# david8862/tf-keras-speech-commands

Hardware: AMD Instinct MI355X
Metric: 1 s@16 kHz clips/sec train-step, simple_cnn bs4096, 1/2/4/8 MI355X; eval top-1 (higher is better)
Workload: dtype f32; 1 GPU; configs[1]: simple_cnn train step = featurize(f32 1 s @16 kHz) + fwd + bwd + Adam, 36 logits (background + 35 words), batch 4096 per GPU; global_batch=4096, parallelism=dp1, gradient_exchange=none (one rank), rccl_ranks=0, library_build=546ca62dfe01

## Files before the change

### tf-keras-speech-commands_amd/csrc/kws_cnn_plan.h

```cpp
#pragma once
#include "kws_model_types.h"
#include "kws_layers.h"
#include "kws_layer1.h"
#include "kws_infer_fused.h"
#include "kws_conv_group.h"
#include "kws_dense_head.h"

namespace kws {

struct CnnPlan {
    bool training, bf16, det;
    bool prepared;
    bool fused_tail;
    bool group;
    bool dense_fused;
    bool l1m;
    bool l1_default_map;
    bool prep_in_stats;
    bool l1_conv2;
    bool compact_g2;
    bool routed_g2;
    bool fuse_pool2;
    bool acc_fwd;
    bool acc_bn2, acc_bn3, acc_bn4;
    bool a3_on_load;
    bool pool4_fused;
    bool wgrad2_bf16;
    bool wgrad2_early;
    bool l1_fin_in_kernel;
    bool head_bwd_fuses;
    bool fuse_head_fwd;
};

inline CnnPlan plan_cnn(const kws_model *m, int B, int mprec, bool training, bool capturing, bool wants_head_outputs, bool prepared)
{
    const CnnDims &d = m->d;
    CnnPlan p{};
    p.training = training;
    p.bf16 = mprec == 1;
    p.det = m->deterministic != 0;
    p.prepared = !training && prepared;
    const bool split_train = p.bf16 && training;
    const bool default_tail = m->kind == KWS_SIMPLE_CNN && d.H2 == kFuH2 && d.W2 == kFuW2 && d.H3 == kFuH3 && d.W3 == kFuW3;
    p.fused_tail = !training && wants_head_outputs && p.bf16 && default_tail && d.H4 == kFuH4 && d.W4 == kFuW4 && m->C <= kFuHeadCols;
    p.group = split_train && default_tail && (long)blocks_for(B, kFuClips) <= kStatStride;
    p.head_bwd_fuses = head_bwd_fuses(m);
    p.fuse_head_fwd = p.head_bwd_fuses && !p.det;
    p.dense_fused = split_train && m->kind == KWS_SIMPLE_CNN && p.fuse_head_fwd && m->head_K == kDhK && d.flat % (16 * kDhWaves) == 0 && d.flat <= 1024;
    p.l1m = d.H0 % 2 == 0 && d.W0 % 2 == 0 && (d.H0 + 2) * (d.W0 + 2) <= 64 * kL1Stage && (d.H0 / 2) * (d.W0 / 2) <= 4 * kL1MaxTiles;
    p.l1_default_map = d.H0 == 30 && d.W0 == 20;
    p.prep_in_stats = split_train && p.l1m;
    const int P1 = d.H1 * d.W1;
    p.compact_g2 = p.bf16 && P1 * 8 <= 1280 && (size_t)(d.H1 / 2) * (d.W1 / 2) * 32 <= sizeof(float) * (size_t)d.H3 * d.W3 * 64;
    p.routed_g2 = p.compact_g2;
    p.fuse_pool2 = p.group && p.routed_g2 && d.H1 == kGrH1 && d.W1 == kGrW1;
    const bool acc_ok = !p.det && !capturing;
    p.acc_fwd = p.fuse_pool2 && acc_ok;
    p.l1_conv2 = p.prep_in_stats && p.acc_fwd && p.l1_default_map;
    p.a3_on_load = split_train;
    p.pool4_fused = p.acc_fwd && p.dense_fused;
    p.wgrad2_bf16 = p.bf16 && P1 <= 160;
    p.wgrad2_early = p.compact_g2 && p.wgrad2_bf16 && P1 * 8 <= 1280 && P1 * 4 <= 768;
    p.acc_bn2 = p.group && acc_ok && p.routed_g2 && p.wgrad2_early;
    p.acc_bn3 = p.group && acc_ok;
    p.acc_bn4 = p.dense_fused && acc_ok && d.flat == d.H4 * d.W4 * kDhK;
    p.l1_fin_in_kernel = acc_ok && p.l1_default_map;
    return p;
}

}
```

### tf-keras-speech-commands_amd/csrc/kws_model.hip

```cpp
#include <cstdlib>
#include <cstring>
#include <string>
#include <vector>

#include "kws_common.h"
#include "kws_model_types.h"
#include "kws_conv.h"
#include "kws_layers.h"
#include "kws_layer1.h"
#include "kws_layer1_moments.h"
#include "kws_layer1_fast.h"
#include "kws_l1_conv2.h"
#include "kws_lite.h"
#include "kws_lite_f16.h"
#include "kws_infer_fused.h"
#include "kws_conv_group.h"
#include "kws_dense_head.h"
#include "kws_cnn_plan.h"

using namespace kws;

namespace {

inline int same_out(int n, int s) { return (n + s - 1) / s; }
inline int same_pad_before(int n, int k, int s)
{
    const int out = same_out(n, s), total = std::max((out - 1) * s + k - n, 0);
    return total / 2;
}

struct OverlapHook {
    hipEvent_t ev = nullptr;
    void (*cb)(void *) = nullptr;
    void *user = nullptr;
    int at = 0;
    bool fired = false;
    bool wants(int point) const { return !fired && point == at; }
    int fire(int point, hipStream_t s, bool already_bound = false)
    {
        if (fired || point != at) return KWS_OK;
        fired = true;
        if (ev && !already_bound) KWS_HIP_CHECK(hipEventRecord(ev, s));
        if (cb) cb(user);
        return KWS_OK;
    }
};

#define KWS_TRY_NB(...)               \
    do {                              \
        const int rc__ = (__VA_ARGS__); \
        if (rc__ < 0) return rc__;    \
    } while (0)
#define KWS_TRY(...)                  \
    do {                              \
        if (int rc__ = (__VA_ARGS__)) return rc__; \
    } while (0)

constexpr int kCh[5] = {1, 16, 32, 64, 128};
constexpr int kMaxStatBlocks = kStatStride;

struct CnnWs {
    float *z[4], *a[4], *d1, *loss_i, *correct_i, *dlogits, *dd1, *da4, *gz[4], *da[3];
    float *dwo[4], *ddw[4];
    float *coef[4];
    __bf16 *wsp[3][6];
    __bf16 *dzp[3];
    double *partial;
    double *moments;
    float *zmax2;
    unsigned char *arg2;
    float *zmax4;
    unsigned char *arg4;
    unsigned char *base;
    size_t bytes;
};

CnnWs carve_cnn(const kws_model *m, int B, bool training, unsigned char *base)
{
    CnnWs w{};
    w.base = base;
    size_t off = 0;
    auto take = [&](size_t nfloats) {
        float *p = reinterpret_cast<float *>(base + off);
        off = al256(off + nfloats * sizeof(float));
        return p;
    };
    const CnnDims &d = m->d;
    const size_t zs[4] = {(size_t)d.H0 * d.W0 * 16, (size_t)d.H1 * d.W1 * 32, (size_t)d.H3 * d.W3 * 64, (size_t)d.H3 * d.W3 * 128};
    const size_t as[4] = {(size_t)d.H1 * d.W1 * 16, (size_t)d.H2 * d.W2 * 32, (size_t)d.H3 * d.W3 * 64, (size_t)d.flat};
    const bool lite = m->kind == KWS_SIMPLE_CNN_LITE;
    const size_t dws[4] = {(size_t)d.H0 * d.W0 * 1, (size_t)d.H1 * d.W1 * 16, (size_t)d.H3 * d.W3 * 32, (size_t)d.H3 * d.W3 * 64};
    for (int i = 0; i < 4; ++i) { w.z[i] = take((i == 0 && !lite) ? 0 : zs[i] * B); w.a[i] = take(as[i] * B); }
    for (int i = 0; i < 4; ++i) w.dwo[i] = take(lite ? dws[i] * B : 0);
    w.d1 = take((size_t)B * 128);
    w.loss_i = take(B);
    w.correct_i = take(B);
    for (int i = 0; i < 4; ++i) w.coef[i] = take(6 * 128);
    {
        const size_t wn[3] = {(size_t)9 * 32 * 64, (size_t)9 * 64 * 128, (size_t)d.flat * 128};
        for (int t = 0; t < 3; ++t)
            for (int q = 0; q < 6; ++q) w.wsp[t][q] = reinterpret_cast<__bf16 *>(take(lite ? 0 : (wn[t] + 1) / 2));
    }
    w.partial = reinterpret_cast<double *>(take((size_t)kMaxStatBlocks * 9 * 64 * 2));
    w.moments = reinterpret_cast<double *>(take(2 * kMomCount));
    if (training) {
        w.dlogits = take((size_t)B * m->C);
        w.dd1 = take((size_t)B * 128);
        w.da4 = take((size_t)B * d.flat);
        for (int i = 0; i < 4; ++i) w.gz[i] = take((i == 0 && !lite) ? 0 : zs[i] * B);
        for (int p = 0; p < 3; ++p) w.dzp[p] = reinterpret_cast<__bf16 *>(take(lite ? 0 : (zs[3] * B + 1) / 2));
        for (int i = 0; i < 4; ++i) w.ddw[i] = take(lite ? dws[i] * B : 0);
        for (int i = 0; i < 3; ++i) w.da[i] = take(as[i] * B);
        w.zmax2 = take(lite ? 0 : as[1] * B);
        w.arg2 = reinterpret_cast<unsigned char *>(take(lite ? 0 : (as[1] * B + 3) / 4));
        w.zmax4 = take(lite ? 0 : as[3] * B);
        w.arg4 = reinterpret_cast<unsigned char *>(take(lite ? 0 : (as[3] * B + 3) / 4));
    }
    w.bytes = off;
    return w;
}

BnCoef coef_of(float *base, int C) { return BnCoef{base, base + C, base + 2 * C, base + 3 * C, base + 4 * C, base + 5 * C}; }
static double *acc_set(ModelRes *R, int pass, int layer, unsigned parity) { return R->acc + ((size_t)(pass * 4 + layer) * 2 + (parity & 1u)) * kAccDoubles; }
static int acc_make_clean(ModelRes *R, hipStream_t s)
{
    if (R->acc_dirty) {
        KWS_HIP_CHECK(hipMemsetAsync(R->acc, 0, sizeof(double) * 2 * 4 * 2 * kAccDoubles, s));
        R->acc_dirty = false;
    }
    return KWS_OK;
}

static int infer_coefs(const kws_model *m, const float *params, const float *state, CnnWs &w, hipStream_t s)
{
    BnInferAll a;
    for (int l = 0; l < 4; ++l) {
        a.C[l] = kCh[l + 1];
        a.gamma[l] = params + m->o_g[l]; a.beta[l] = params + m->o_b[l];
        a.mm[l] = state + m->o_mm[l]; a.mv[l] = state + m->o_mv[l];
        a.k[l] = coef_of(w.coef[l], kCh[l + 1]);
    }
    KWS_LAUNCH("bn_infer_coef_all_kernel", bn_infer_coef_all_kernel, dim3(4), dim3(128), 0, s, a);
    return KWS_OK;
}

inline void stat_grid(long M, int C, int &nblk, int &rows)
{
    const int R = 256 / C;
    long want = (M + (long)R * 8 - 1) / ((long)R * 8);
    nblk = (int)std::min<long>(kMaxStatBlocks, std::max<long>(1, want));
    rows = (int)((M + nblk - 1) / nblk);
    nblk = (int)((M + rows - 1) / rows);
}

template <int CR, int CO, int MODE, int EPI>
int launch_gemm(const float *src, const float *w, const float *bias, float *dst, const ConvGeom &g, hipStream_t s)
{
    const long M = (long)g.B * g.Ho * g.Wo;
    static const std::string name = std::string("conv_gemm_fwd<") + std::to_string(CR) + "," +
                                    std::to_string(CO) + ">";
    KWS_LAUNCH(name.c_str(), (conv_gemm_kernel<CR, CO, MODE, EPI>), dim3(blocks_for(M, 64)), dim3(256), 0, s, src, w, bias, dst, g);
    return KWS_OK;
}

static int cu_count() { return device_cus(); }
// ... 598 lines not shown
    } else
        KWS_TRY(run_head_bwd(m, B, params, w.d1, w.dlogits, w.dd1, grads, true, s, nullptr, w.loss_i, w.correct_i,
                             stats, P.det));
    const bool fork0_bound = stop_event_bound(fork0_ev);
    if (P.fuse_head_fwd) {
        if (a->forward_event) KWS_HIP_CHECK(hipEventRecord(static_cast<hipEvent_t>(a->forward_event), s));
        if (hook) KWS_TRY(hook->fire(1, s));
    }
    const ConvGeom g = dense_geom(d, B);
    const bool hook_ev_here = hook && hook->wants(2) && hook->ev;
    if (hook) KWS_TRY(hook->fire(2, s, fork0_bound && hook_ev_here));
    if (hook_ev_here) {
        KWS_HIP_CHECK(hipStreamWaitEvent(s2, fork0_ev, 0));
    } else {
        if (!fork0_bound) KWS_HIP_CHECK(hipEventRecord(R->ev[0], s));
        KWS_HIP_CHECK(hipStreamWaitEvent(s2, R->ev[0], 0));
    }
    if (P.fuse_head_fwd && stats) KWS_LAUNCH("loss_reduce_kernel", loss_reduce_kernel, dim3(1), dim3(256), 0, s2, w.loss_i, w.correct_i, B, stats);
    KWS_TRY(launch_wgrad<128, 128, 1>(w.a[3], w.dd1, grads + m->o_dk, g, s2, P.det));
    if (!P.fuse_head_fwd) {
        int nblk, rows;
        stat_grid(B, 128, nblk, rows);
        KWS_LAUNCH("channel_stats_kernel.dense", channel_stats_kernel, dim3(nblk), dim3(256), 0, s, w.dd1, (long)B, 128, rows, w.partial);
        KWS_LAUNCH("colsum_finalize_kernel", colsum_finalize_kernel, dim3(128), dim3(256), 0, s, w.partial, nblk, 128, grads + m->o_db);
    }
    if (P.dense_fused) ;
    else if (P.bf16) KWS_TRY_NB(launch_bf16<128, 128, MODE_DGRAD, EPI_NONE>("conv_bf16_dgrad", w.dd1, w.wsp[2], nullptr, w.da4, g, s));
    else KWS_TRY(launch_dgrad<128, 128, 1>(w.dd1, params + m->o_dk, w.da4, g, s));
    if (hook) KWS_TRY(hook->fire(3, s));
    return KWS_OK;
}

int CnnCtx::bwd_layer4()
{
    const int C = 128, H = d.H3, W = d.W3;
    const long M = pixels(3);
    const BnCoef k = coef(3);
    const float *gamma = params + m->o_g[3];
    const float rate = drop_rate();
    int nblk, rows;
    stat_grid((long)B * (H / 2) * (W / 2), C, nblk, rows);
    if (P.acc_bn4) ;
    else if (P.bf16)
        KWS_LAUNCH(prof_name("bn_bwd_reduce_pool_kernel", 4), bn_bwd_reduce_routed_full_kernel, dim3(nblk), dim3(256), 0, s, w.zmax4, w.arg4, w.da4, k,
                   w.gz[3], B, H, W, C, rows, w.partial, rate, slo(), shi());
    else KWS_TRY(bwd_reduce_pool(3, H, W, C, w.da4, rate, nblk, rows));
    if (!P.acc_bn4) KWS_TRY(bwd_bn_finalize(3, C, nblk));
    bwd_arm(3);
    const Bf16PlanesOut dzp{{w.dzp[0], w.dzp[1], w.dzp[2]}};
    if (P.acc_bn4)
        KWS_LAUNCH(prof_name("bn_bwd_apply_planes_kernel", 4), bn_bwd_apply_routed_planes_kernel<true>, dim3(std::min<unsigned>(1024u, blocks_for(M * C / 4, 256))),
                   dim3(256), 0, s, w.z[3], w.da4, w.arg4, k, gamma, B, H, W, C, acc_out(3), dzp);
    else if (P.bf16)
        KWS_LAUNCH(prof_name("bn_bwd_apply_planes_kernel", 4), bn_bwd_apply_planes_kernel<true>, dim3(blocks_for(M * C / 4, 256)), dim3(256), 0, s,
                   w.z[3], w.gz[3], k, gamma, M * C / 4, C, dzp);
    else
        KWS_LAUNCH(prof_name("bn_bwd_apply_kernel", 4), bn_bwd_apply_kernel<true>, dim3(blocks_for(M * C, 256)), dim3(256), 0, s, w.z[3], w.gz[3], k,
                   gamma, M * C, C);
    if (hook) KWS_TRY(hook->fire(4, s));
    KWS_TRY(bwd_fork(3));
    const float *in = w.a[2], *kern = params + m->o_k[3];
    float *dk = grads + m->o_k[3];
    const ConvGeom g = geom3x3(B, H, W, 1);
    if (P.bf16 && P.a3_on_load)
        KWS_TRY((launch_wgrad_bf16<64, 128, 1, true, true>(w.z[2], nullptr, dk, g, s2, w.dzp, P.det, coef(2).scale)));
    else if (P.bf16) KWS_TRY(launch_wgrad_bf16<64, 128, 1, true>(in, nullptr, dk, g, s2, w.dzp, P.det));
    else KWS_TRY(launch_wgrad<64, 128, 1>(in, w.gz[3], dk, g, s2, P.det));
    if (a->comm) KWS_TRY(comm_allreduce_early(a->comm, grads + m->o_k[3], m->P - m->o_k[3], s2));
    if (a->bucket_event) KWS_HIP_CHECK(hipEventRecord(static_cast<hipEvent_t>(a->bucket_event), s2));
    if (P.group) {
        fused_bn3_blocks = launch_group_dgrad4(m, B, w, s, P.acc_bn3 ? acc_set(R, 1, 2, bpar[2]) : nullptr);
        if (fused_bn3_blocks < 0) return fused_bn3_blocks;
    } else if (P.bf16 && blocks_for(M, 64) <= (unsigned)kStatStride) {
        const BnCoef k3 = coef(2);
        fused_bn3_blocks = launch_bf16<128, 64, MODE_DGRAD, EPI_BNBWD_GATE6>("conv_bf16_dgrad", nullptr, w.wsp[1], k3.scale, w.gz[2], g, s, w.partial,
                                                                             w.z[2], w.dzp);
        if (fused_bn3_blocks < 0) return fused_bn3_blocks;
    } else if (P.bf16)
        KWS_TRY_NB(launch_bf16<128, 64, MODE_DGRAD, EPI_NONE>("conv_bf16_dgrad", nullptr, w.wsp[1], nullptr, w.da[2], g, s, nullptr, nullptr, w.dzp));
    else KWS_TRY(launch_dgrad<128, 64, 1>(w.gz[3], kern, w.da[2], g, s));
    return KWS_OK;
}

int CnnCtx::bwd_layer3()
{
    const int C = 64, H = d.H3, W = d.W3;
    if (hook) KWS_TRY(hook->fire(5, s));
    const long M = pixels(2);
    const BnCoef k = coef(2);
    const float *gamma = params + m->o_g[2];
    int nblk, rows;
    stat_grid(M, C, nblk, rows);
    if (fused_bn3_blocks > 0) nblk = fused_bn3_blocks;
    else
        KWS_LAUNCH(prof_name("bn_bwd_reduce_kernel", 3), bn_bwd_reduce_kernel<false>, dim3(nblk), dim3(256), 0, s, w.z[2], w.da[2], k, w.gz[2], B, H, W, C,
                   rows, w.partial, 0.f, slo(), shi());
    if (!P.acc_bn3) KWS_TRY(bwd_bn_finalize(2, C, nblk));
    bwd_arm(2);
    if (P.acc_bn3)
        KWS_LAUNCH(prof_name("bn_bwd_apply_kernel", 3), bn_bwd_apply_acc_kernel<false>, dim3(std::min<unsigned>(1024u, blocks_for(M * C / 4, 256))), dim3(256), 0, s,
                   w.z[2], w.gz[2], k, gamma, M * C / 4, C, acc_out(2));
    else
        KWS_LAUNCH(prof_name("bn_bwd_apply_kernel", 3), bn_bwd_apply_kernel<false>, dim3(blocks_for(M * C, 256)), dim3(256), 0, s, w.z[2], w.gz[2], k,
                   gamma, M * C, C);
    KWS_TRY(bwd_fork(2));
    const float *in = w.a[1], *kern = params + m->o_k[2];
    float *dk = grads + m->o_k[2];
    const ConvGeom g = geom3x3(B, d.H2, d.W2, 2);
    if (P.bf16) KWS_TRY(launch_wgrad_bf16<32, 64, 3>(in, w.gz[2], dk, g, s2, nullptr, P.det));
    else KWS_TRY(launch_wgrad<32, 64, 3>(in, w.gz[2], dk, g, s2, P.det));
    if (P.group) {
        if (P.acc_bn2) bwd_arm(1);
        KWS_TRY(launch_group_dgrad3(m, B, w, s, P.acc_bn2 ? acc_set(R, 1, 1, bpar[1]) : nullptr));
    }
    else KWS_TRY(launch_dgrad<64, 32, 2>(w.gz[2], kern, w.da[1], g, s));
    return KWS_OK;
}

int CnnCtx::bwd_layer2()
{
    const int C = 32, H1 = d.H1, W1 = d.W1;
    const long M = pixels(1);
    const BnCoef k = coef(1);
    const long NW = (long)B * (H1 / 2) * (W1 / 2);
    int nblk, rows;
    stat_grid(NW, C, nblk, rows);
    if (P.acc_bn2) ;
    else if (P.compact_g2 && P.routed_g2)
        KWS_LAUNCH(prof_name("bn_bwd_reduce_pool_kernel", 2), bn_bwd_reduce_routed_kernel, dim3(nblk), dim3(256), 0, s, w.zmax2, w.da[1], k, NW, C,
                   rows, w.partial);
    else if (P.compact_g2)
        KWS_LAUNCH(prof_name("bn_bwd_reduce_pool_kernel", 2), bn_bwd_reduce_pool_kernel<true>, dim3(nblk), dim3(256), 0, s, w.z[1], w.da[1], k,
                   w.gz[1], B, H1, W1, C, rows, w.partial, 0.f, slo(), shi(), reinterpret_cast<unsigned char *>(w.da[2]));
    else KWS_TRY(bwd_reduce_pool(1, H1, W1, C, w.da[1], 0.f, nblk, rows));
    if (!P.acc_bn2) {
        if (P.wgrad2_early) bwd_arm(1);
        KWS_TRY(bwd_bn_finalize(1, C, nblk));
    }
    const float *in = w.a[0], *kern = params + m->o_k[1];
    float *dk = grads + m->o_k[1];
    const Conv2Clip cc = conv2_clip(d, B);
    BnBwdArgs bn = {w.z[1], params + m->o_g[1], k.mean, k.inv, k.k2, k.k3};
    if (P.compact_g2) { bn.gw = w.da[1]; bn.arg = P.routed_g2 ? w.arg2 : reinterpret_cast<const unsigned char *>(w.da[2]); }
    BnBwdArgs bn_w = bn;
    if (P.acc_bn2) {
        bn.acc = bn_w.acc = acc_set(R, 1, 1, bpar[1]);
        bn.M = bn_w.M = M;
        bn.acc_clear_set = acc_set(R, 1, 1, bpar[1] + 1);
        bn.dgamma = grads + m->o_g[1]; bn.dbeta = grads + m->o_b[1]; bn.k2w = k.k2; bn.k3w = k.k3;
    }
    auto wgrad_grid = [&](int occ) { return dim3(P.det ? 1u : cc.even_grid(cu_count() * std::min(occ, 2))); };
    if (P.wgrad2_early) {
        KWS_TRY(bwd_fork(1));
        static const int occ = resident_blocks(conv_wgrad_clip_bf16_kernel<true>, 256, cc.smwb);
        arm_stop_event(R->ev[9], s2);
        KWS_LAUNCH("conv_wgrad_clip_bf16<16,32>", conv_wgrad_clip_bf16_kernel<true>, wgrad_grid(occ), dim3(256), cc.smwb, s2, in, nullptr, dk, B, H1, W1, bn_w);
    }
    if (P.bf16) {
        const dim3 grid(cc.even_grid(cu_count() * 2));
        if (P.wgrad2_early)
            KWS_LAUNCH("conv_dgrad_clip_bf16<32,16>", (conv_dgrad_clip_bf16_kernel<true, true, false>), grid, dim3(256), cc.smdb, s,
                       w.gz[1], kern, w.da[0], B, H1, W1, bn);
        else if (P.compact_g2)
            KWS_LAUNCH("conv_dgrad_clip_bf16<32,16>", (conv_dgrad_clip_bf16_kernel<true, true>), grid, dim3(256), cc.smdb, s,
                       w.gz[1], kern, w.da[0], B, H1, W1, bn);
        else
            KWS_LAUNCH("conv_dgrad_clip_bf16<32,16>", (conv_dgrad_clip_bf16_kernel<true, false>), grid, dim3(256), cc.smdb, s,
                       w.gz[1], kern, w.da[0], B, H1, W1, bn);
    } else
        KWS_LAUNCH("conv_dgrad_clip<32,16>", (conv_dgrad_clip_kernel<32, true>), dim3(cc.even_grid(cu_count() * 5)), dim3(256), cc.smd, s, w.gz[1], kern, w.da[0],
                   B, H1, W1, bn);
    if (P.wgrad2_early) return KWS_OK;
    KWS_TRY(bwd_fork(1));
    if (P.wgrad2_bf16) {
        static const int occ = resident_blocks(conv_wgrad_clip_bf16_kernel<false>, 256, cc.smwb);
        KWS_LAUNCH("conv_wgrad_clip_bf16<16,32>", conv_wgrad_clip_bf16_kernel<false>, wgrad_grid(occ), dim3(256), cc.smwb, s2, in, w.gz[1], dk, B, H1, W1, bn);
    } else
        KWS_LAUNCH("conv_wgrad_clip<16,32>", conv_wgrad_clip_kernel<32>, dim3(P.det ? 1u : cc.even_grid(cu_count() * 3)), dim3(256), cc.smw, s2, in, w.gz[1], dk,
                   B, H1, W1);
    return KWS_OK;
}

int CnnCtx::bwd_layer1()
{
    const L1Geom g = l1_geom(d, B, P);
    BnCoef k1 = coef(0);
    const float *kern1 = params + m->o_k[0];
    if (P.l1m) {
        const double *q = moments ? moments : w.moments;
        if (P.l1_fin_in_kernel) {
            double *acc0 = acc_set(R, 1, 0, 0);
            const L1FinalizeArgs fin{acc0, reinterpret_cast<unsigned *>(acc0 + kAccDoubles - 1), q, params + m->o_g[0], grads + m->o_k[0],
                                     grads + m->o_g[0], grads + m->o_b[0]};
            KWS_LAUNCH("l1m_bwd_onepass_kernel", (l1f_bwd_onepass_kernel<30, 20>), dim3(g.nbm), dim3(256), g.smemm, s, feat, kern1, w.da[0], k1, B, g.cpw, w.partial, fin);
        } else if (P.l1_default_map)
            KWS_LAUNCH("l1m_bwd_onepass_kernel", (l1f_bwd_onepass_kernel<30, 20>), dim3(g.nbm), dim3(256), g.smemm, s, feat, kern1, w.da[0], k1, B, g.cpw, w.partial);
        else
            KWS_LAUNCH("l1m_bwd_onepass_kernel", l1m_bwd_onepass_kernel, dim3(g.nbm), dim3(256), g.smemm, s, feat, kern1, w.da[0], k1, B, d.H0, d.W0, g.cpw,
                       w.partial);
        if (!P.l1_fin_in_kernel)
            KWS_LAUNCH("l1_bwd_finalize_moments_kernel", l1_bwd_finalize_moments_kernel, dim3(144 + 16), dim3(64), 0, s, w.partial, g.nbm, q, kern1,
                       params + m->o_g[0], k1, grads + m->o_k[0], grads + m->o_g[0], grads + m->o_b[0]);
    } else {
        KWS_LAUNCH("l1_bwd_reduce_kernel", l1_bwd_reduce_kernel<16>, dim3(g.nb), dim3(256), g.smem1, s, feat, kern1, w.da[0], k1, B, d.H0, d.W0,
                   g.cpb, w.partial);
        KWS_TRY(bwd_bn_finalize(0, 16, g.nb));
        KWS_LAUNCH("l1_bwd_wgrad_kernel", l1_bwd_wgrad_kernel<16>, dim3(P.det ? 1 : g.nb), dim3(256), g.smem1, s, feat, kern1, w.da[0], k1, params + m->o_g[0],
                   grads + m->o_k[0], B, d.H0, d.W0, P.det ? B : g.cpb);
    }
    return KWS_OK;
}

int CnnCtx::backward()
{
    const DisarmOnExit disarm_guard;
    if (!P.bf16) KWS_HIP_CHECK(hipMemsetAsync(grads, 0, sizeof(float) * (size_t)m->P, s));
    bpar[1] = P.acc_bn2 ? R->acc_uses[1][1]++ : 0u;
    bpar[2] = P.acc_bn3 ? R->acc_uses[1][2]++ : 0u;
    bpar[3] = P.acc_bn4 ? R->acc_uses[1][3]++ : 0u;
    KWS_TRY(acc_make_clean(R, s));
    R->acc_dirty = true;
    KWS_TRY(bwd_head_dense());
    KWS_TRY(bwd_layer4());
    KWS_TRY(bwd_layer3());
    KWS_TRY(bwd_layer2());
    KWS_TRY(bwd_layer1());
    if (!stop_event_bound(R->ev[9])) KWS_HIP_CHECK(hipEventRecord(R->ev[9], s2));
    KWS_HIP_CHECK(hipStreamWaitEvent(s, R->ev[9], 0));
    KWS_LAUNCH_CHECK("simple_cnn backward");
    R->acc_dirty = false;
    return KWS_OK;
}


ConvGeom geom1x1(int B, int H, int W)
{
    ConvGeom g;
    g.B = B; g.H = H; g.W = W; g.Ho = H; g.Wo = W; g.stride = 1; g.pt = 0; g.pl = 0; g.KH = 1; g.KW = 1;
    return g;
}


static int lite_forward_f16(const kws_model *m, const float *feat, int B, const float *params, const float *state, CnnWs &w, float *probs,
                            int32_t *argmax, hipStream_t s)
{
    const CnnDims &d = m->d;
    const bool front_ok = d.H0 % 2 == 0 && d.W0 % 2 == 0 && (d.H0 + 2) * (d.W0 + 2) <= 64 * 12 && d.H2 >= 1 && d.W2 >= 1;
    if (!front_ok || d.H2 * d.W2 > kF16MaxN2 || d.H3 * d.W3 > kF16MaxP3 || d.H4 < 1 || d.W4 < 1 || m->C > kF16HeadCols || d.flat > kWdRow)
        return fail(KWS_ERR_UNSUPPORTED, "fp16 inference of simple_cnn_lite needs a feature map up to about 30 x 20 and at most %d classes "
                                         "(got %d x %d, %d classes): use KWS_INFER_FP32", kF16HeadCols, d.H0, d.W0, m->C);
    const bool prepared = m->prepared_for(params, state, w.base, B, matrix_prec(m), infer_prec(m));
    _Float16 *blob = reinterpret_cast<_Float16 *>(w.partial);
    if (!prepared) {
        if (int rc = infer_coefs(m, params, state, w, s)) return rc;
        KWS_LAUNCH("lite_f16_prepare_kernel", lite_f16_prepare_kernel, dim3(32), dim3(256), 0, s, params + m->o_pwk[2], params + m->o_pwk[3],
                   params + m->o_dk, params + m->o_hk, m->C, d.flat, blob);
    }
    BnCoef k0 = coef_of(w.coef[0], 16), k1 = coef_of(w.coef[1], 32), k2 = coef_of(w.coef[2], 64), k3 = coef_of(w.coef[3], 128);
    const LiteFrontArgs fa = {params + m->o_dwk[0], params + m->o_pwk[0], params + m->o_pwb[0], k0.scale, k0.shift,
                              params + m->o_dwk[1], params + m->o_pwk[1], params + m->o_pwb[1], k1.scale, k1.shift};
    const size_t sm = sizeof(float) * (size_t)lite_front_floats(d.H0, d.W0);
    const int waves = cu_count() * std::max(1, std::min(8, (int)(160 * 1024 / sm)));
    const int cpw = std::max(1, (B + waves - 1) / waves), nblk = (B + cpw - 1) / cpw;
    _Float16 *a2h = reinterpret_cast<_Float16 *>(w.a[1]);
    KWS_LAUNCH("lite_front_infer_kernel", lite_front_infer_kernel, dim3(nblk), dim3(64), sm, s, feat, fa, w.a[1], B, d.H0, d.W0, cpw, a2h);
    LiteF16Args a;
    a.dwk3 = params + m->o_dwk[2]; a.pwb3 = params + m->o_pwb[2]; a.sc3 = k2.scale; a.sh3 = k2.shift;
    a.dwk4 = params + m->o_dwk[3]; a.pwb4 = params + m->o_pwb[3]; a.sc4 = k3.scale; a.sh4 = k3.shift;
    a.db = params + m->o_db; a.hb = params + m->o_hb; a.blob = blob;
    a.C = m->C; a.H2 = d.H2; a.W2 = d.W2; a.H3 = d.H3; a.W3 = d.W3;
    a.pt3 = same_pad_before(d.H2, 3, 2); a.pl3 = same_pad_before(d.W2, 3, 2); a.H4 = d.H4; a.W4 = d.W4;
    if (int rc = ensure_dynamic_lds(reinterpret_cast<const void *>(lite_back_f16_kernel), kF16LdsBytes)) return rc;
    const int ntile = (B + kF16Clips - 1) / kF16Clips;
    KWS_LAUNCH("lite_back_f16_kernel", lite_back_f16_kernel, dim3(std::min(ntile, cu_count())), dim3(256), (size_t)kF16LdsBytes, s, a2h, a, B, probs, argmax);
    KWS_LAUNCH_CHECK("simple_cnn_lite fp16 forward");
    return KWS_OK;
}

int lite_forward(const kws_model *m, const float *feat, int B, const float *params, float *state, CnnWs &w, bool training,
                 uint64_t seed, hipStream_t s)
{
    const CnnDims &d = m->d;
    const int Hs[4] = {d.H0, d.H1, d.H2, d.H3}, Ws[4] = {d.W0, d.W1, d.W2, d.W3};
    const int Hz[4] = {d.H0, d.H1, d.H3, d.H3}, Wz[4] = {d.W0, d.W1, d.W3, d.W3};
    const int strd[4] = {1, 1, 2, 1};
    const bool pool[4] = {true, true, false, true};
    const uint32_t slo = (uint32_t)(seed & 0xFFFFFFFFu), shi = (uint32_t)(seed >> 32);
    int l_begin = 0;
    if (!training && !m->prepared_for(params, state, w.base, B, matrix_prec(m), infer_prec(m)))
        if (int rc = infer_coefs(m, params, state, w, s)) return rc;
    if (!training && d.H0 % 2 == 0 && d.W0 % 2 == 0 && (d.H0 + 2) * (d.W0 + 2) <= 64 * 12 && d.H2 >= 1 && d.W2 >= 1) {
        BnCoef k0 = coef_of(w.coef[0], 16), k1 = coef_of(w.coef[1], 32);
        const LiteFrontArgs fa = {params + m->o_dwk[0], params + m->o_pwk[0], params + m->o_pwb[0], k0.scale, k0.shift,
                                  params + m->o_dwk[1], params + m->o_pwk[1], params + m->o_pwb[1], k1.scale, k1.shift};
        const size_t sm = sizeof(float) * (size_t)lite_front_floats(d.H0, d.W0);
        const int waves = cu_count() * std::max(1, std::min(8, (int)(160 * 1024 / sm)));
        const int cpw = std::max(1, (B + waves - 1) / waves), nblk = (B + cpw - 1) / cpw;
        KWS_LAUNCH("lite_front_infer_kernel", lite_front_infer_kernel, dim3(nblk), dim3(64), sm, s, feat, fa, w.a[1], B, d.H0, d.W0, cpw);
        l_begin = 2;
    }
    for (int l = l_begin; l < 4; ++l) {
        const float *in = l == 0 ? feat : w.a[l - 1];
        const int Cin = kCh[l], C = kCh[l + 1];
        const long M = (long)B * Hz[l] * Wz[l];
        const ConvGeom g = geom3x3(B, Hs[l], Ws[l], strd[l]);
        KWS_LAUNCH(prof_name("dwconv_fwd_kernel", l + 1), dwconv_fwd_kernel, dim3(blocks_for(M * Cin, 256)), dim3(256), 0, s, in,
                   params + m->o_dwk[l], w.dwo[l], g, Cin);
        const float *pwk = params + m->o_pwk[l], *pwb = params + m->o_pwb[l];
        const ConvGeom g1 = geom1x1(B, Hz[l], Wz[l]);
// ... 575 lines not shown
```

Baseline: 7.748 million clips/s.

## Add specialized pipelined MFMA kernel for conv2 weight gradient at 15x10 maps

Adds a dedicated conv2 weight-gradient kernel for the default 15x10 map. Each wave streams clips through a ring buffer of three input rows in LDS, split into three bf16 planes. The BN-backward and pool-routing gradient is recomputed on load and fed into MFMA accumulations, with the next clip's loads overlapped with the current products. It replaces the generic clip wgrad kernel when the early bf16 wgrad and accumulated-BN plan flags hold. This adds a large shape-specific code path, and the per-block atomic reduction could add contention.

```diff
diff --git a/tf-keras-speech-commands_amd/csrc/kws_cnn_plan.h b/tf-keras-speech-commands_amd/csrc/kws_cnn_plan.h
--- a/tf-keras-speech-commands_amd/csrc/kws_cnn_plan.h
+++ b/tf-keras-speech-commands_amd/csrc/kws_cnn_plan.h
@@ -5,6 +5,8 @@
 #include "kws_infer_fused.h"
 #include "kws_conv_group.h"
 #include "kws_dense_head.h"
+#include "kws_conv.h"
+#include "kws_conv2_wgrad_fast.h"
 
 namespace kws {
 
@@ -27,6 +29,7 @@
     bool pool4_fused;
     bool wgrad2_bf16;
     bool wgrad2_early;
+    bool wgrad2_fast;
     bool l1_fin_in_kernel;
     bool head_bwd_fuses;
     bool fuse_head_fwd;
@@ -65,6 +68,7 @@
     p.acc_bn3 = p.group && acc_ok;
     p.acc_bn4 = p.dense_fused && acc_ok && d.flat == d.H4 * d.W4 * kDhK;
     p.l1_fin_in_kernel = acc_ok && p.l1_default_map;
+    p.wgrad2_fast = p.wgrad2_early && p.acc_bn2 && d.H1 == kW2fH && d.W1 == kW2fW;
     return p;
 }
 
diff --git a/tf-keras-speech-commands_amd/csrc/kws_conv2_wgrad_fast.h b/tf-keras-speech-commands_amd/csrc/kws_conv2_wgrad_fast.h
--- /dev/null
+++ b/tf-keras-speech-commands_amd/csrc/kws_conv2_wgrad_fast.h
@@ -0,0 +1,224 @@
+#pragma once
+
+namespace kws {
+
+constexpr int kW2fH = 15, kW2fW = 10;
+
+template <int H, int W>
+struct Conv2WgradFast {
+    static constexpr int CIN = 16, COUT = 32, RS = 3, KS = H / RS, RING = 2 * RS, WP = W + 2, HW = H * W, KP = RS * W;
+    static constexpr int RB = WP * 32, XPL = RING * RB, DPL = 32 * 32;
+    static constexpr int XBYTES = 3 * XPL, WAVE_BYTES = XBYTES + 6 * DPL, BYTES = 4 * WAVE_BYTES;
+    static constexpr int NX4 = (RS + 1) * W * 4;
+    static_assert(H % RS == 0 && KS >= 2 && W % 2 == 0 && KP <= 32 && KP > 24, "a k-step is three whole map rows, 25..32 pixels");
+    static_assert(NX4 <= 192 && WAVE_BYTES % 16 == 0, "three float4 of x per lane");
+    static_assert(BYTES >= 4 * 9 * CIN * COUT, "the block's tile fits the staging space");
+    static unsigned grid(int B, int max_blocks) { const int cpw = (B + 4 * max_blocks - 1) / (4 * max_blocks); return (unsigned)((B + 4 * cpw - 1) / (4 * cpw)); }
+};
+
+template <int H, int W>
+__global__ __launch_bounds__(256, 2) void conv2_wgrad_fast_kernel(const float *__restrict__ x, float *__restrict__ dw, int B, BnBwdArgs bn)
+{
+    using G = Conv2WgradFast<H, W>;
+    constexpr int CIN = G::CIN, COUT = G::COUT, RS = G::RS, KS = G::KS, RING = G::RING, HW = G::HW, KP = G::KP;
+    constexpr int RB = G::RB, XPL = G::XPL, DPL = G::DPL, Wp = W / 2, NWIN = (H / 2) * Wp, F4 = COUT / 4;
+    extern __shared__ __attribute__((aligned(16))) unsigned char ctile[];
+    const int lane = threadIdx.x & 63, wave = __builtin_amdgcn_readfirstlane(threadIdx.x >> 6), li = lane & 15, lq = lane >> 4;
+    unsigned char *Xs = ctile + wave * G::WAVE_BYTES, *Ds = Xs + G::XBYTES;
+#pragma unroll
+    for (int j = 0; j < (G::WAVE_BYTES / 16 + 63) / 64; ++j) {
+        const int i = lane + 64 * j;
+        if (i < G::WAVE_BYTES / 16) reinterpret_cast<f32x4 *>(Xs)[i] = (f32x4){0.f, 0.f, 0.f, 0.f};
+    }
+
+    __shared__ __attribute__((aligned(16))) float coef[5][COUT];
+    const int c4 = lane & (F4 - 1), l8 = lane >> 3;
+    {
+        f32x4 gi, mean, inv;
+        float k2[4], k3[4];
+#pragma unroll
+        for (int e = 0; e < 4; ++e) {
+            const int c = 4 * c4 + e;
+            inv[e] = bn.inv[c]; gi[e] = bn.gamma[c] * inv[e]; mean[e] = bn.mean[c];
+        }
+        bn_bwd_k_from_acc(bn, COUT, c4, false, k2, k3);
+        if (threadIdx.x < F4) {
+            *reinterpret_cast<f32x4 *>(&coef[0][4 * c4]) = gi;
+            *reinterpret_cast<f32x4 *>(&coef[1][4 * c4]) = mean;
+            *reinterpret_cast<f32x4 *>(&coef[2][4 * c4]) = inv;
+            *reinterpret_cast<f32x4 *>(&coef[3][4 * c4]) = (f32x4){k2[0], k2[1], k2[2], k2[3]};
+            *reinterpret_cast<f32x4 *>(&coef[4][4 * c4]) = (f32x4){k3[0], k3[1], k3[2], k3[3]};
+        }
+        __syncthreads();
+    }
+
+    int xa[2][3][2], da[2];
+#pragma unroll
+    for (int rd = 0; rd < 2; ++rd) {
+        const int pq = 16 * rd + 4 * lq + (li >> 2);
+        const bool ok = pq < KP;
+        const int ly = ok ? pq / W : 0, lx = ok ? pq - ly * W : 0;
+        da[rd] = pq * 32 + (li & 3) * 8;
+#pragma unroll
+        for (int par = 0; par < 2; ++par)
+#pragma unroll
+            for (int kh = 0; kh < 3; ++kh) xa[par][kh][rd] = ((RS * par + ly + kh) % RING) * RB + lx * 32 + (li & 3) * 8;
+    }
+    int dly[4], dlx[4], xry[3], xof[3];
+#pragma unroll
+    for (int j = 0; j < 4; ++j) { const int pix = l8 + 8 * j; dly[j] = pix / W; dlx[j] = pix - dly[j] * W; }
+#pragma unroll
+    for (int j = 0; j < 3; ++j) { const int i = lane + 64 * j, xp = i >> 2; xry[j] = xp / W; xof[j] = (xp - xry[j] * W + 1) * 32 + (i & 3) * 8; }
+    const int dso = ((c4 >> 2) * 32 + l8) * 32 + (c4 & 3) * 8;
+
+    auto frag = [&](const unsigned char *p0, const unsigned char *p1) -> bf16x8 {
+        union { struct { s16x4 lo, hi; } s; bf16x8 v; } u;
+        u.s.lo = lds_read_tr16(p0);
+        u.s.hi = lds_read_tr16(p1);
+        return u.v;
+    };
+
+    f32x4 acc[9][2];
+#pragma unroll
+    for (int t = 0; t < 9; ++t) acc[t][0] = acc[t][1] = (f32x4){0.f, 0.f, 0.f, 0.f};
+
+    f32x4 rx[3], rz[4], rg[4];
+    unsigned ra[4];
+    auto first = [](int k) { return k == 0 ? 0 : RS * k + 1; };
+    auto rows = [&](int k) { return k == 0 ? RS + 1 : (H - first(k) < RS ? H - first(k) : RS); };
+    auto load = [&](int k, long b) {
+        const int nx4 = rows(k) * W * 4;
+        const f32x4 *xs = reinterpret_cast<const f32x4 *>(x + (b * HW + first(k) * W) * CIN);
+#pragma unroll
+        for (int j = 0; j < 3; ++j) {
+            const int i = lane + 64 * j;
+            if (64 * j < nx4) rx[j] = i < nx4 ? xs[i] : (f32x4){0.f, 0.f, 0.f, 0.f};
+        }
+        const f32x4 *zs = reinterpret_cast<const f32x4 *>(bn.z + (b * HW + KP * k) * COUT);
+        const f32x4 *gws = reinterpret_cast<const f32x4 *>(bn.gw) + b * NWIN * F4;
+        const unsigned *ars = reinterpret_cast<const unsigned *>(bn.arg) + b * NWIN * F4;
+#pragma unroll
+        for (int j = 0; j < 4; ++j) {
+            const int y = RS * k + dly[j];
+            const bool ok = l8 + 8 * j < KP, in = ok && y < 2 * (H / 2);
+            const int q = in ? ((y >> 1) * Wp + (dlx[j] >> 1)) * F4 + c4 : 0;
+            rg[j] = gws[q];
+            ra[j] = ars[q];
+            rz[j] = ok ? zs[lane + 64 * j] : (f32x4){0.f, 0.f, 0.f, 0.f};
+        }
+    };
+    auto put = [&](unsigned char *d, int plane_bytes, f32x4 v) {
+        bf16x4 h, m, l;
+        split_bf16(v, h, m, l);
+        *reinterpret_cast<bf16x4 *>(d) = h;
+        *reinterpret_cast<bf16x4 *>(d + plane_bytes) = m;
+        *reinterpret_cast<bf16x4 *>(d + 2 * plane_bytes) = l;
+    };
+    auto zero_row = [&](int slot) {
+        if (lane < 3 * W * 2)
+            *reinterpret_cast<f32x4 *>(Xs + (lane / (2 * W)) * XPL + slot * RB + 32 + (lane % (2 * W)) * 16) = (f32x4){0.f, 0.f, 0.f, 0.f};
+    };
+    auto stage = [&](int k) {
+        const int nx4 = rows(k) * W * 4, s0 = (first(k) + 1) % RING;
+#pragma unroll
+        for (int j = 0; j < 3; ++j) {
+            const int i = lane + 64 * j;
+            if (64 * j < nx4 && i < nx4) {
+                int slot = s0 + xry[j];
+                slot -= slot >= RING ? RING : 0;
+                put(Xs + slot * RB + xof[j], XPL, rx[j]);
+            }
+        }
+        if (k == 0) zero_row(0);
+        if (k == KS - 1) zero_row((H + 1) % RING);
+        const f32x4 gi = *reinterpret_cast<const f32x4 *>(&coef[0][4 * c4]), mean = *reinterpret_cast<const f32x4 *>(&coef[1][4 * c4]),
+                    inv = *reinterpret_cast<const f32x4 *>(&coef[2][4 * c4]), k2 = *reinterpret_cast<const f32x4 *>(&coef[3][4 * c4]),
+                    k3 = *reinterpret_cast<const f32x4 *>(&coef[4][4 * c4]);
+#pragma unroll
+        for (int j = 0; j < 4; ++j) {
+            if (l8 + 8 * j < KP) {
+                const int y = RS * k + dly[j], ce = (y & 1) * 2 + (dlx[j] & 1);
+                const bool in = y < 2 * (H / 2);
+                f32x4 v = rg[j];
+#pragma unroll
+                for (int e = 0; e < 4; ++e) {
+                    const float g = (in && (int)((ra[j] >> (8 * e)) & 0xFFu) == ce) ? v[e] : 0.f;
+                    v[e] = gi[e] * (g - k2[e] - (rz[j][e] - mean[e]) * inv[e] * k3[e]);
+                }
+                put(Ds + dso + j * 8 * 32, 2 * DPL, v);
+            }
+        }
+    };
+    auto products = [&](int k) {
+        const int par = k & 1;
+        bf16x8 bfr[2][3];
+#pragma unroll
+        for (int nt = 0; nt < 2; ++nt)
+#pragma unroll
+            for (int p = 0; p < 3; ++p) bfr[nt][p] = frag(Ds + (2 * p + nt) * DPL + da[0], Ds + (2 * p + nt) * DPL + da[1]);
+        auto xfrag = [&](int tap, bf16x8 (&a)[3]) {
+            const int kh = tap / 3, kw = tap % 3;
+#pragma unroll
+            for (int p = 0; p < 3; ++p) a[p] = frag(Xs + p * XPL + kw * 32 + xa[par][kh][0], Xs + p * XPL + kw * 32 + xa[par][kh][1]);
+        };
+        bf16x8 a[2][3];
+        xfrag(0, a[0]);
+#pragma unroll
+        for (int tap = 0; tap < 9; ++tap) {
+            if (tap + 1 < 9) xfrag(tap + 1, a[(tap + 1) & 1]);
+            constexpr int pa[6] = {1, 2, 0, 1, 0, 0}, pb[6] = {1, 0, 2, 0, 1, 0};
+#pragma unroll
+            for (int i = 0; i < 6; ++i) {
+                acc[tap][0] = mfma_bf16(a[tap & 1][pa[i]], bfr[0][pb[i]], acc[tap][0]);
+                acc[tap][1] = mfma_bf16(a[tap & 1][pa[i]], bfr[1][pb[i]], acc[tap][1]);
+            }
+            __builtin_amdgcn_sched_barrier(0);
+        }
+    };
+
+    const long stride = 4L * gridDim.x;
+    long b = 4L * blockIdx.x + wave;
+    if (b < B) {
+        load(0, b);
+        stage(0);
+    }
+    for (; b < B; b += stride) {
+#pragma unroll
+        for (int j = 0; j < 4; ++j) asm volatile("" : "+v"(dly[j]), "+v"(dlx[j]));
+#pragma unroll
+        for (int j = 0; j < 3; ++j) asm volatile("" : "+v"(xry[j]), "+v"(xof[j]));
+#pragma unroll
+        for (int k = 0; k < KS; ++k) {
+            const bool wrap = k == KS - 1;
+            const int nk = wrap ? 0 : k + 1;
+            const long nb = wrap ? b + stride : b;
+            __builtin_amdgcn_fence(__ATOMIC_ACQ_REL, "wavefront");
+            if (nb < B) load(nk, nb);
+            __builtin_amdgcn_sched_barrier(0);
+            products(k);
+            __builtin_amdgcn_fence(__ATOMIC_ACQ_REL, "wavefront");
+            if (nb < B) stage(nk);
+        }
+    }
+
+    float *red = reinterpret_cast<float *>(ctile);
+#pragma unroll
+    for (int w = 0; w < 4; ++w) {
+        __syncthreads();
+        if (wave == w) {
+#pragma unroll
+            for (int tap = 0; tap < 9; ++tap)
+#pragma unroll
+                for (int nt = 0; nt < 2; ++nt)
+#pragma unroll
+                    for (int r = 0; r < 4; ++r) {
+                        float *p = red + (tap * CIN + 4 * lq + r) * COUT + 16 * nt + li;
+                        *p = w == 0 ? acc[tap][nt][r] : *p + acc[tap][nt][r];
+                    }
+        }
+    }
+    __syncthreads();
+    for (int idx = threadIdx.x; idx < 9 * CIN * COUT; idx += 256) atomicAdd(dw + idx, red[idx]);
+}
+
+}
diff --git a/tf-keras-speech-commands_amd/csrc/kws_model.hip b/tf-keras-speech-commands_amd/csrc/kws_model.hip
--- a/tf-keras-speech-commands_amd/csrc/kws_model.hip
+++ b/tf-keras-speech-commands_amd/csrc/kws_model.hip
@@ -11,6 +11,7 @@
 #include "kws_layer1_moments.h"
 #include "kws_layer1_fast.h"
 #include "kws_l1_conv2.h"
+#include "kws_conv2_wgrad_fast.h"
 #include "kws_lite.h"
 #include "kws_lite_f16.h"
 #include "kws_infer_fused.h"
@@ -915,9 +916,16 @@
     auto wgrad_grid = [&](int occ) { return dim3(P.det ? 1u : cc.even_grid(cu_count() * std::min(occ, 2))); };
     if (P.wgrad2_early) {
         KWS_TRY(bwd_fork(1));
-        static const int occ = resident_blocks(conv_wgrad_clip_bf16_kernel<true>, 256, cc.smwb);
         arm_stop_event(R->ev[9], s2);
-        KWS_LAUNCH("conv_wgrad_clip_bf16<16,32>", conv_wgrad_clip_bf16_kernel<true>, wgrad_grid(occ), dim3(256), cc.smwb, s2, in, nullptr, dk, B, H1, W1, bn_w);
+        if (P.wgrad2_fast) {
+            using G = Conv2WgradFast<kW2fH, kW2fW>;
+            if (int rc = ensure_dynamic_lds(reinterpret_cast<const void *>(conv2_wgrad_fast_kernel<kW2fH, kW2fW>), G::BYTES)) return rc;
+            KWS_LAUNCH("conv_wgrad_clip_bf16<16,32>", (conv2_wgrad_fast_kernel<kW2fH, kW2fW>), dim3(G::grid(B, cu_count() * 2)), dim3(256), G::BYTES, s2, in, dk,
+                       B, bn_w);
+        } else {
+            static const int occ = resident_blocks(conv_wgrad_clip_bf16_kernel<true>, 256, cc.smwb);
+            KWS_LAUNCH("conv_wgrad_clip_bf16<16,32>", conv_wgrad_clip_bf16_kernel<true>, wgrad_grid(occ), dim3(256), cc.smwb, s2, in, nullptr, dk, B, H1, W1, bn_w);
+        }
     }
     if (P.bf16) {
         const dim3 grid(cc.even_grid(cu_count() * 2));
```

New measurement: 7.929 million clips/s, median of 6. 1.02x the previous value.
